# ed-fish/data-efficient-video-transformers

Hardware: AMD Instinct MI355X
Metric: clips/sec fwd+bwd, B=8 T=32 3x224x224 bf16 (higher is better)
Workload: dtype bf16; 1 GPU; ViViT metric shape (SURVEY 8 'M'; BASELINE configs[2]/[3] transformer): B=8/GPU, T=32, 3x224x224, patch 16, d=512, ...; global_batch=8, parallelism=dp1

## Files before the change

data-efficient-video-transformers_amd/csrc/attention.hip:

```cpp
#include "common.h"
#include <cstdlib>

namespace {

__device__ __forceinline__ void wave_lds_sync() {
  asm volatile("s_waitcnt lgkmcnt(0)" ::: "memory");
  __builtin_amdgcn_wave_barrier();
}

constexpr float kLog2e = 1.4426950408889634f;
constexpr float kLn2 = 0.6931471805599453f;

struct AttnParams {
  const void *q, *k, *v, *o, *d_o;
  void *out, *dq, *dk, *dv;
  float* lse;
  float* delta;
  int B, H, Lq, Lk, dh;
  int64_t q_sb, q_sh, q_sl, k_sb, k_sh, k_sl, v_sb, v_sh, v_sl, o_sb, o_sh, o_sl;
  float scale;
  int Lkp;
  int Lqp;
  int patch_off;
  uint32_t drop_thr;
  float drop_scale;
  const uint64_t* rng;
  uint64_t rng_off;
};


__device__ __forceinline__ float attn_drop(const AttnParams& p, int b, int h, int i, int j) {
  if (p.drop_thr == 0u) return 1.0f;
  const uint64_t idx = (((uint64_t)b * p.H + h) * p.Lq + i) * (uint64_t)p.Lk + j;
  return dvt_dropout_keep(p.rng[0], p.rng[1] + p.rng_off, idx, p.drop_thr) ? p.drop_scale : 0.0f;
}

template <typename T>
__global__ __launch_bounds__(256) void attn_fwd_generic_kernel(const AttnParams p) {
  extern __shared__ __attribute__((aligned(16))) float lds_f[];
  const int lane = threadIdx.x & 63, wid = threadIdx.x >> 6;
  float* qs = lds_f + (size_t)wid * (p.dh + p.Lk);
  float* ps = qs + p.dh;
  const int64_t row = (int64_t)blockIdx.x * 4 + wid;
  const int64_t total = (int64_t)p.B * p.H * p.Lq;
  if (row >= total) return;
  const int i = (int)(row % p.Lq);
  const int h = (int)((row / p.Lq) % p.H);
  const int b = (int)(row / ((int64_t)p.Lq * p.H));
  const T* q = (const T*)p.q + b * p.q_sb + h * p.q_sh + (int64_t)i * p.q_sl;
  const T* k = (const T*)p.k + b * p.k_sb + h * p.k_sh;
  const T* v = (const T*)p.v + b * p.v_sb + h * p.v_sh;
  T* o = (T*)p.out + b * p.o_sb + h * p.o_sh + (int64_t)i * p.o_sl;
  for (int e = lane; e < p.dh; e += 64) qs[e] = to_f32<T>(q[e]);
  wave_lds_sync();
  float m = -INFINITY;
  for (int j = lane; j < p.Lk; j += 64) {
    const T* kj = k + (int64_t)j * p.k_sl;
    float s = 0.f;
    for (int e = 0; e < p.dh; ++e) s = fmaf(qs[e], to_f32<T>(kj[e]), s);
    s *= p.scale;
    ps[j] = s;
    m = fmaxf(m, s);
  }
  m = wave_max(m);
  float l = 0.f;
  for (int j = lane; j < p.Lk; j += 64) {
    const float e = expf(ps[j] - m);
    ps[j] = e * attn_drop(p, b, h, i, j);
    l += e;
  }
  l = wave_sum(l);
  wave_lds_sync();
  const float inv = 1.0f / l;
  for (int e = lane; e < p.dh; e += 64) {
    float acc = 0.f;
    for (int j = 0; j < p.Lk; ++j) acc = fmaf(ps[j], to_f32<T>(v[(int64_t)j * p.v_sl + e]), acc);
    o[e] = from_f32<T>(acc * inv);
  }
  if (lane == 0) p.lse[row] = m + logf(l);
}

template <typename T>
__global__ __launch_bounds__(256) void attn_delta_kernel(const AttnParams p) {
  const int lane = threadIdx.x & 63, wid = threadIdx.x >> 6;
  const int64_t row = (int64_t)blockIdx.x * 4 + wid;
  const int64_t total = (int64_t)p.B * p.H * p.Lq;
  if (row >= total) return;
  const int i = (int)(row % p.Lq);
  const int h = (int)((row / p.Lq) % p.H);
  const int b = (int)(row / ((int64_t)p.Lq * p.H));
  const int64_t off = b * p.o_sb + h * p.o_sh + (int64_t)i * p.o_sl;
  const T* o = (const T*)p.o + off;
  const T* g = (const T*)p.d_o + off;
  float s = 0.f;
  for (int e = lane; e < p.dh; e += 64) s = fmaf(to_f32<T>(o[e]), to_f32<T>(g[e]), s);
  s = wave_sum(s);
  if (lane == 0) p.delta[row] = s;
}

template <typename T>
__global__ __launch_bounds__(256) void attn_bwd_dq_generic_kernel(const AttnParams p) {
  extern __shared__ __attribute__((aligned(16))) float lds_f[];
  const int lane = threadIdx.x & 63, wid = threadIdx.x >> 6;
  float* qs = lds_f + (size_t)wid * (2 * p.dh + p.Lk);
  float* gs = qs + p.dh;
  float* ds = gs + p.dh;
  const int64_t row = (int64_t)blockIdx.x * 4 + wid;
  const int64_t total = (int64_t)p.B * p.H * p.Lq;
  if (row >= total) return;
  const int i = (int)(row % p.Lq);
  const int h = (int)((row / p.Lq) % p.H);
  const int b = (int)(row / ((int64_t)p.Lq * p.H));
  const T* q = (const T*)p.q + b * p.q_sb + h * p.q_sh + (int64_t)i * p.q_sl;
  const T* g = (const T*)p.d_o + b * p.o_sb + h * p.o_sh + (int64_t)i * p.o_sl;
  const T* k = (const T*)p.k + b * p.k_sb + h * p.k_sh;
  const T* v = (const T*)p.v + b * p.v_sb + h * p.v_sh;
  T* dq = (T*)p.dq + b * p.q_sb + h * p.q_sh + (int64_t)i * p.q_sl;
  for (int e = lane; e < p.dh; e += 64) {
    qs[e] = to_f32<T>(q[e]);
    gs[e] = to_f32<T>(g[e]);
  }
  wave_lds_sync();
  const float lse = p.lse[row], delta = p.delta[row];
  for (int j = lane; j < p.Lk; j += 64) {
    const T* kj = k + (int64_t)j * p.k_sl;
    const T* vj = v + (int64_t)j * p.v_sl;
    float s = 0.f, dp = 0.f;
    for (int e = 0; e < p.dh; ++e) {
      s = fmaf(qs[e], to_f32<T>(kj[e]), s);
      dp = fmaf(gs[e], to_f32<T>(vj[e]), dp);
    }
    const float pr = expf(s * p.scale - lse);
    ds[j] = pr * (dp * attn_drop(p, b, h, i, j) - delta) * p.scale;
  }
  wave_lds_sync();
  for (int e = lane; e < p.dh; e += 64) {
    float acc = 0.f;
    for (int j = 0; j < p.Lk; ++j) acc = fmaf(ds[j], to_f32<T>(k[(int64_t)j * p.k_sl + e]), acc);
    dq[e] = from_f32<T>(acc);
  }
}

template <typename T>
__global__ __launch_bounds__(256) void attn_bwd_dkv_generic_kernel(const AttnParams p) {
  extern __shared__ __attribute__((aligned(16))) float lds_f[];
  const int lane = threadIdx.x & 63, wid = threadIdx.x >> 6;
  float* ks = lds_f + (size_t)wid * (2 * p.dh + 2 * p.Lq);
  float* vs = ks + p.dh;
  float* ps = vs + p.dh;
  float* ds = ps + p.Lq;
  const int64_t row = (int64_t)blockIdx.x * 4 + wid;
  const int64_t total = (int64_t)p.B * p.H * p.Lk;
  if (row >= total) return;
  const int j = (int)(row % p.Lk);
// ... 797 lines not shown
          const f32x2 ds = pr * d;
          s[tt][r] = ds[0];
          s[tt][r + 1] = ds[1];
          if (last && (2 * kp + tt) * 16 + 4 * g + r >= p.Lk) s[tt][r] = 0.f;
          if (last && (2 * kp + tt) * 16 + 4 * g + r + 1 >= p.Lk) s[tt][r + 1] = 0.f;
        }
      const V8 dsf = pack_pair<E>(s[0], s[1]);
#pragma unroll
      for (int dt = 0; dt < 4; ++dt)
        acc[dt] = Elem16<E>::mma(img_tr_frag<E>(ks, 2 * kp, 2 * kp + 1, dt * 16, g, li), dsf, acc[dt]);
    };
    if constexpr (NKP > 0) {
#pragma unroll
      for (int kp = 0; kp < NKP; ++kp) step(kp, kp == NKP - 1);
    } else {
      for (int kp = 0; kp < nkp - 1; ++kp) step(kp, false);
      step(nkp - 1, true);
    }
#pragma unroll
    for (int kk = 0; kk < 2; ++kk) {
      consume(qn[kk]);
      consume(gn[kk]);
      consume(of[kk]);
    }
    consume(l2n);
    store_tile<E>(patch, dqb, p.q_sl, qt * 16, p.Lq, acc, p.scale, lane);
#pragma unroll
    for (int kk = 0; kk < 2; ++kk) {
      qf[kk] = qn[kk];
      gf[kk] = gn[kk];
    }
    l2 = l2n;
  }
}

template <typename E, int NQP>
__global__ __launch_bounds__(1024) void attn_bwd_dkv_mfma_kernel(const AttnParams p) {
  extern __shared__ __attribute__((aligned(16))) char smem[];
  using V8 = typename Elem16<E>::v8;
  const int lane = threadIdx.x & 63, wid = threadIdx.x >> 6, W = blockDim.x >> 6;
  const int g = lane >> 4, li = lane & 15;
  const int b = blockIdx.x / p.H, h = blockIdx.x % p.H;
  const E* qb = (const E*)p.q + b * p.q_sb + h * p.q_sh;
  const E* kb = (const E*)p.k + b * p.k_sb + h * p.k_sh;
  const E* vb = (const E*)p.v + b * p.v_sb + h * p.v_sh;
  const E* gb = (const E*)p.d_o + b * p.o_sb + h * p.o_sh;
  E* dkb = (E*)p.dk + b * p.k_sb + h * p.k_sh;
  E* dvb = (E*)p.dv + b * p.v_sb + h * p.v_sh;
  const float* lse = p.lse + ((int64_t)b * p.H + h) * p.Lq;
  const float* delta = p.delta + ((int64_t)b * p.H + h) * p.Lq;
  char* qs = smem;
  char* gs = smem + p.Lqp * kRowBytes;
  float* l2s = reinterpret_cast<float*>(smem + 2 * p.Lqp * kRowBytes);
  float* dls = l2s + p.Lqp;
  const int nkt = (p.Lk + 15) >> 4, nqp = NQP ? NQP : p.Lqp >> 5;
  auto load_rows = [&](int kt, V8* kf, V8* vf) {
    const int kj = kt * 16 + li;
    const int krow = kj < p.Lk ? kj : p.Lk - 1;
#pragma unroll
    for (int kk = 0; kk < 2; ++kk) {
      kf[kk] = *reinterpret_cast<const V8*>(kb + (int64_t)krow * p.k_sl + kk * 32 + g * 8);
      vf[kk] = *reinterpret_cast<const V8*>(vb + (int64_t)krow * p.v_sl + kk * 32 + g * 8);
    }
  };
  V8 kf[2], vf[2];
  load_rows(wid, kf, vf);
  const int sr = (int)threadIdx.x < p.Lq ? (int)threadIdx.x : p.Lq - 1;
  const float lse0 = lse[sr], dl0 = delta[sr];
  stage_images<E>(qs, qb, p.q_sl, gs, gb, p.o_sl, p.Lq, p.Lqp);
  if ((int)threadIdx.x < p.Lqp) {
    l2s[threadIdx.x] = (int)threadIdx.x < p.Lq ? -lse0 * kLog2e : 0.f;
    dls[threadIdx.x] = (int)threadIdx.x < p.Lq ? -dl0 : 0.f;
  }
  for (int r = threadIdx.x + blockDim.x; r < p.Lqp; r += blockDim.x) {
    l2s[r] = r < p.Lq ? -lse[r] * kLog2e : 0.f;
    dls[r] = r < p.Lq ? -delta[r] : 0.f;
  }
  __syncthreads();

  const float c2 = p.scale * kLog2e;
  char* patch = p.patch_off >= 0 ? smem + p.patch_off + wid * 2048 : nullptr;
  for (int kt = wid; kt < nkt; kt += W) {
    asm volatile("" ::: "memory");
    f32x4 dk[4], dv[4];
#pragma unroll
    for (int dt = 0; dt < 4; ++dt) {
      dk[dt] = f32x4{0.f, 0.f, 0.f, 0.f};
      dv[dt] = f32x4{0.f, 0.f, 0.f, 0.f};
    }
    const f32x2 c2v = {c2, c2};
    auto step = [&](int qp) {
      f32x4 s[2], dp[2];
#pragma unroll
      for (int tt = 0; tt < 2; ++tt) {
        s[tt] = f32x4{0.f, 0.f, 0.f, 0.f};
        dp[tt] = f32x4{0.f, 0.f, 0.f, 0.f};
#pragma unroll
        for (int kk = 0; kk < 2; ++kk) {
          s[tt] = Elem16<E>::mma(img_row_frag<E>(qs, (2 * qp + tt) * 16, kk, g, li), kf[kk], s[tt]);
          dp[tt] = Elem16<E>::mma(img_row_frag<E>(gs, (2 * qp + tt) * 16, kk, g, li), vf[kk], dp[tt]);
        }
      }
#pragma unroll
      for (int tt = 0; tt < 2; ++tt) {
        const int q0 = (2 * qp + tt) * 16 + 4 * g;
        const f32x4 l2 = *reinterpret_cast<const f32x4*>(l2s + q0);
        const f32x4 dl = *reinterpret_cast<const f32x4*>(dls + q0);
#pragma unroll
        for (int r = 0; r < 4; r += 2) {
          const f32x2 x = __builtin_elementwise_fma(f32x2{s[tt][r], s[tt][r + 1]}, c2v, f32x2{l2[r], l2[r + 1]});
          const f32x2 d = f32x2{dp[tt][r], dp[tt][r + 1]} + f32x2{dl[r], dl[r + 1]};
          const f32x2 pr = {__builtin_amdgcn_exp2f(x[0]), __builtin_amdgcn_exp2f(x[1])};
          const f32x2 ds = pr * d;
          s[tt][r] = pr[0];
          s[tt][r + 1] = pr[1];
          dp[tt][r] = ds[0];
          dp[tt][r + 1] = ds[1];
        }
      }
      const V8 pf = pack_pair<E>(s[0], s[1]);
      const V8 dsf = pack_pair<E>(dp[0], dp[1]);
#pragma unroll
      for (int dt = 0; dt < 4; ++dt) {
        dv[dt] = Elem16<E>::mma(img_tr_frag<E>(gs, 2 * qp, 2 * qp + 1, dt * 16, g, li), pf, dv[dt]);
        dk[dt] = Elem16<E>::mma(img_tr_frag<E>(qs, 2 * qp, 2 * qp + 1, dt * 16, g, li), dsf, dk[dt]);
      }
    };
    if constexpr (NQP > 0) {
#pragma unroll
      for (int qp = 0; qp < NQP; ++qp) step(qp);
    } else {
      for (int qp = 0; qp < nqp; ++qp) step(qp);
    }
    if (kt + W < nkt) load_rows(kt + W, kf, vf);
    store_tile<E>(patch, dkb, p.k_sl, kt * 16, p.Lk, dk, p.scale, lane);
    store_tile<E>(patch, dvb, p.v_sl, kt * 16, p.Lk, dv, 1.0f, lane);
  }
}

constexpr int kStripRow = 80;

template <typename E>
__device__ __forceinline__ typename Elem16<E>::v8 strip_tr_frag(const char* strip, int ta, int tb, int col0, int g, int li) {
  const int qq = li >> 2, pp = li & 3;
  typename Elem16<E>::v4 half[2];
#pragma unroll
  for (int hf = 0; hf < 2; ++hf) {
    const int r = 16 * (hf ? tb : ta) + 4 * g + qq;
    half[hf] = Elem16<E>::tr_read(strip + r * kStripRow + col0 * 2 + 8 * pp);
  }
  return __builtin_shufflevector(half[0], half[1], 0, 1, 2, 3, 4, 5, 6, 7);
}

template <typename E, int NCH>
__device__ __forceinline__ void stage_bwd_operands(char* qs, const E* q, int64_t q_sl, char* gs, const E* g, const E* o, int64_t o_sl,
                                                   char* ks, const E* k, int64_t k_sl, int Lq, int Lk, int rows_pad, float* dls) {
  using V8 = typename Elem16<E>::v8;
  const int total = rows_pad * 8, nt = blockDim.x;
  V8 vq[NCH], vg[NCH], vo[NCH], vk[NCH];
#pragma unroll
  for (int u = 0; u < NCH; ++u) {
    const int idx = min((int)threadIdx.x + u * nt, total - 1);
    const int r = idx >> 3, c = idx & 7;
    const int rq = r < Lq ? r : 0, rk = r < Lk ? r : 0;
    vq[u] = *reinterpret_cast<const V8*>(q + (int64_t)rq * q_sl + c * 8);
    vg[u] = *reinterpret_cast<const V8*>(g + (int64_t)rq * o_sl + c * 8);
    vo[u] = *reinterpret_cast<const V8*>(o + (int64_t)rq * o_sl + c * 8);
    vk[u] = *reinterpret_cast<const V8*>(k + (int64_t)rk * k_sl + c * 8);
  }
  __builtin_amdgcn_sched_barrier(0);
  const V8 zero = {0, 0, 0, 0, 0, 0, 0, 0};
#pragma unroll
  for (int u = 0; u < NCH; ++u) {
    const int idx = min((int)threadIdx.x + u * nt, total - 1);
    const int r = idx >> 3, off = img_off(r, idx & 7);
    const bool lq = r < Lq, lk = r < Lk;
    *reinterpret_cast<V8*>(qs + off) = lq ? vq[u] : zero;
    *reinterpret_cast<V8*>(gs + off) = lq ? vg[u] : zero;
    *reinterpret_cast<V8*>(ks + off) = lk ? vk[u] : zero;
    float d = 0.f;
#pragma unroll
    for (int j = 0; j < 8; ++j) d = fmaf((float)vg[u][j], (float)vo[u][j], d);
    d += __shfl_xor(d, 1, 64);
    d += __shfl_xor(d, 2, 64);
    d += __shfl_xor(d, 4, 64);
    if ((idx & 7) == 0) dls[r] = lq ? -d : 0.f;
  }
}

template <typename E, int NP>
__global__ __launch_bounds__(512) void attn_bwd_fused_kernel(const AttnParams p) {
  extern __shared__ __attribute__((aligned(16))) char smem[];
  using V8 = typename Elem16<E>::v8;
  using V4 = typename Elem16<E>::v4;
  constexpr int LP = 32 * NP;
  const int lane = threadIdx.x & 63;
  const int wid = __builtin_amdgcn_readfirstlane(threadIdx.x >> 6);
  const int W = blockDim.x >> 6, WC = W - 1;
  const int g = lane >> 4, li = lane & 15;
  const int b = blockIdx.x / p.H, h = blockIdx.x % p.H;
  const E* qb = (const E*)p.q + b * p.q_sb + h * p.q_sh;
  const E* kb = (const E*)p.k + b * p.k_sb + h * p.k_sh;
  const E* vb = (const E*)p.v + b * p.v_sb + h * p.v_sh;
  const E* ob = (const E*)p.o + b * p.o_sb + h * p.o_sh;
  const E* gb = (const E*)p.d_o + b * p.o_sb + h * p.o_sh;
  E* dqb = (E*)p.dq + b * p.q_sb + h * p.q_sh;
  E* dkb = (E*)p.dk + b * p.k_sb + h * p.k_sh;
  E* dvb = (E*)p.dv + b * p.v_sb + h * p.v_sh;
  const float* lse = p.lse + ((int64_t)b * p.H + h) * p.Lq;
  char* qs = smem;
  char* gs = qs + LP * kRowBytes;
  char* ks = gs + LP * kRowBytes;
  char* strip0 = ks + LP * kRowBytes;
  float* l2s = reinterpret_cast<float*>(strip0 + 2 * LP * kStripRow);
  float* dls = l2s + LP;
  char* patch = reinterpret_cast<char*>(dls + LP) + wid * 2048;

  V8 kf[2][2], vf[2][2];
  if (wid < WC) {
#pragma unroll
    for (int j = 0; j < 2; ++j) {
      const int kj = (2 * wid + j) * 16 + li;
      const int krow = kj < p.Lk ? kj : p.Lk - 1;
#pragma unroll
      for (int kk = 0; kk < 2; ++kk) {
        kf[j][kk] = *reinterpret_cast<const V8*>(kb + (int64_t)krow * p.k_sl + kk * 32 + g * 8);
        vf[j][kk] = *reinterpret_cast<const V8*>(vb + (int64_t)krow * p.v_sl + kk * 32 + g * 8);
      }
    }
  }
  {
    const int r = threadIdx.x;
    const float l = lse[r < p.Lq ? r : 0];
    stage_bwd_operands<E, 4>(qs, qb, p.q_sl, gs, gb, ob, p.o_sl, ks, kb, p.k_sl, p.Lq, p.Lk, LP, dls);
    if (r < LP) l2s[r] = r < p.Lq ? -l * kLog2e : 0.f;
  }
  __syncthreads();
  const float c2 = p.scale * kLog2e;
  if (wid < WC) {
    f32x4 dk[2][4], dv[2][4];
#pragma unroll
    for (int j = 0; j < 2; ++j)
#pragma unroll
      for (int dt = 0; dt < 4; ++dt) {
        dk[j][dt] = f32x4{0.f, 0.f, 0.f, 0.f};
        dv[j][dt] = f32x4{0.f, 0.f, 0.f, 0.f};
      }
    const f32x2 c2v = {c2, c2};
    const bool kvalid[2] = {(2 * wid) * 16 + li < p.Lk, (2 * wid + 1) * 16 + li < p.Lk};
    char* myrow[2] = {strip0 + ((2 * wid) * 16 + li) * kStripRow + g * 8, strip0 + ((2 * wid + 1) * 16 + li) * kStripRow + g * 8};
#pragma unroll
    for (int qp = 0; qp < NP; ++qp) {
      asm volatile("" ::: "memory");
      V8 qfr[2][2], gfr[2][2];
#pragma unroll
      for (int tt = 0; tt < 2; ++tt)
#pragma unroll
        for (int kk = 0; kk < 2; ++kk) {
          qfr[tt][kk] = img_row_frag<E>(qs, (2 * qp + tt) * 16, kk, g, li);
          gfr[tt][kk] = img_row_frag<E>(gs, (2 * qp + tt) * 16, kk, g, li);
        }
      f32x4 l2[2], dl[2];
#pragma unroll
      for (int tt = 0; tt < 2; ++tt) {
        l2[tt] = *reinterpret_cast<const f32x4*>(l2s + (2 * qp + tt) * 16 + 4 * g);
        dl[tt] = *reinterpret_cast<const f32x4*>(dls + (2 * qp + tt) * 16 + 4 * g);
      }
      V8 pf[2], dsf[2];
#pragma unroll
      for (int j = 0; j < 2; ++j) {
        f32x4 s[2], dp[2];
#pragma unroll
        for (int tt = 0; tt < 2; ++tt) {
          s[tt] = f32x4{0.f, 0.f, 0.f, 0.f};
          dp[tt] = f32x4{0.f, 0.f, 0.f, 0.f};
#pragma unroll
          for (int kk = 0; kk < 2; ++kk) {
            s[tt] = Elem16<E>::mma(qfr[tt][kk], kf[j][kk], s[tt]);
            dp[tt] = Elem16<E>::mma(gfr[tt][kk], vf[j][kk], dp[tt]);
          }
        }
#pragma unroll
        for (int tt = 0; tt < 2; ++tt)
#pragma unroll
          for (int r = 0; r < 4; r += 2) {
            const f32x2 x = __builtin_elementwise_fma(f32x2{s[tt][r], s[tt][r + 1]}, c2v, f32x2{l2[tt][r], l2[tt][r + 1]});
            const f32x2 d = f32x2{dp[tt][r], dp[tt][r + 1]} + f32x2{dl[tt][r], dl[tt][r + 1]};
            f32x2 pr = {__builtin_amdgcn_exp2f(x[0]), __builtin_amdgcn_exp2f(x[1])};
            if (!kvalid[j]) pr = f32x2{0.f, 0.f};
            const f32x2 ds = pr * d;
            s[tt][r] = pr[0];
            s[tt][r + 1] = pr[1];
            dp[tt][r] = ds[0];
            dp[tt][r + 1] = ds[1];
          }
        pf[j] = pack_pair<E>(s[0], s[1]);
        dsf[j] = pack_pair<E>(dp[0], dp[1]);
      }
#pragma unroll
      for (int j = 0; j < 2; ++j) {
        char* row = myrow[j] + (qp & 1) * (LP * kStripRow);
        *reinterpret_cast<V4*>(row) = __builtin_shufflevector(dsf[j], dsf[j], 0, 1, 2, 3);
        *reinterpret_cast<V4*>(row + 32) = __builtin_shufflevector(dsf[j], dsf[j], 4, 5, 6, 7);
      }
#pragma unroll
      for (int dt = 0; dt < 4; ++dt) {
        const V8 gt = img_tr_frag<E>(gs, 2 * qp, 2 * qp + 1, dt * 16, g, li);
        const V8 qt = img_tr_frag<E>(qs, 2 * qp, 2 * qp + 1, dt * 16, g, li);
#pragma unroll
        for (int j = 0; j < 2; ++j) {
          dv[j][dt] = Elem16<E>::mma(gt, pf[j], dv[j][dt]);
          dk[j][dt] = Elem16<E>::mma(qt, dsf[j], dk[j][dt]);
        }
      }
      __syncthreads();
    }
#pragma unroll
    for (int j = 0; j < 2; ++j) {
      const int k0 = (2 * wid + j) * 16;
      if (k0 < p.Lk) {
        store_tile<E>(patch, dkb, p.k_sl, k0, p.Lk, dk[j], p.scale, lane);
        store_tile<E>(patch, dvb, p.v_sl, k0, p.Lk, dv[j], 1.0f, lane);
      }
    }
  } else {
    V8 ka[NP][4];
#pragma unroll
    for (int kp = 0; kp < NP; ++kp)
#pragma unroll
      for (int dt = 0; dt < 4; ++dt) ka[kp][dt] = img_tr_frag<E>(ks, 2 * kp, 2 * kp + 1, dt * 16, g, li);
#pragma unroll 1
    for (int qp = 0; qp < NP; ++qp) {
      __syncthreads();
      const char* strip = strip0 + (qp & 1) * (LP * kStripRow);
      V8 bq[NP][2];
#pragma unroll
      for (int kp = 0; kp < NP; ++kp) {
        bq[kp][0] = strip_tr_frag<E>(strip, 2 * kp, 2 * kp + 1, 0, g, li);
        bq[kp][1] = strip_tr_frag<E>(strip, 2 * kp, 2 * kp + 1, 16, g, li);
      }
      f32x4 acc[2][4];
#pragma unroll
      for (int tt = 0; tt < 2; ++tt)
#pragma unroll
        for (int dt = 0; dt < 4; ++dt) acc[tt][dt] = f32x4{0.f, 0.f, 0.f, 0.f};
#pragma unroll
      for (int kp = 0; kp < NP; ++kp)
#pragma unroll
        for (int dt = 0; dt < 4; ++dt) {
          acc[0][dt] = Elem16<E>::mma(ka[kp][dt], bq[kp][0], acc[0][dt]);
          acc[1][dt] = Elem16<E>::mma(ka[kp][dt], bq[kp][1], acc[1][dt]);
        }
#pragma unroll
      for (int tt = 0; tt < 2; ++tt)
        if ((2 * qp + tt) * 16 < p.Lq) store_tile<E>(nullptr, dqb, p.q_sl, (2 * qp + tt) * 16, p.Lq, acc[tt], p.scale, lane);
    }
  }
}

constexpr int kMaxLds = 160 * 1024;

int fill_params(const dvt_attn_desc* d, AttnParams& p, bool bwd, const char* name) {
  DVT_REQUIRE(d, "%s: null descriptor", name);
  DVT_REQUIRE(d->q && d->k && d->v && d->o && d->lse, "%s: null q/k/v/o/lse", name);
  DVT_REQUIRE(d->B >= 0 && d->H > 0 && d->Lq > 0 && d->Lk > 0 && d->dh > 0, "%s: bad sizes", name);
  DVT_REQUIRE(d->B * d->H < (1ll << 31) && d->Lq < (1 << 24) && d->Lk < (1 << 24), "%s: sizes too large", name);
  if (bwd) DVT_REQUIRE(d->d_o && d->dq && d->dk && d->dv, "%s: null gradient pointer", name);
  p.q = d->q; p.k = d->k; p.v = d->v; p.o = d->o; p.out = d->o; p.d_o = d->d_o;
  p.dq = d->dq; p.dk = d->dk; p.dv = d->dv; p.lse = d->lse; p.delta = nullptr;
  p.B = (int)d->B; p.H = (int)d->H; p.Lq = (int)d->Lq; p.Lk = (int)d->Lk; p.dh = (int)d->dh;
  p.q_sb = d->q_sb; p.q_sh = d->q_sh; p.q_sl = d->q_sl;
  p.k_sb = d->k_sb; p.k_sh = d->k_sh; p.k_sl = d->k_sl;
  p.v_sb = d->v_sb; p.v_sh = d->v_sh; p.v_sl = d->v_sl;
  p.o_sb = d->o_sb; p.o_sh = d->o_sh; p.o_sl = d->o_sl;
  p.scale = d->scale;
  DVT_REQUIRE(d->dropout_p >= 0.f && d->dropout_p < 1.f, "%s: dropout_p must be in [0, 1)", name);
  DVT_REQUIRE(d->dropout_p == 0.f || d->rng_state, "%s: dropout needs rng_state", name);
  p.drop_thr = 0u; p.drop_scale = 1.f; p.rng = d->rng_state; p.rng_off = d->rng_offset;
  if (d->dropout_p > 0.f) {
    const double th = (double)d->dropout_p * 4294967296.0;
    p.drop_thr = th >= 4294967295.0 ? 0xFFFFFFFFu : (uint32_t)(th + 0.5);
    if (p.drop_thr == 0u) p.drop_thr = 1u;
    p.drop_scale = 1.0f / (1.0f - d->dropout_p);
  }
  p.Lkp = (p.Lk + 31) & ~31;
  p.Lqp = (p.Lq + 31) & ~31;
  p.patch_off = -1;

  return DVT_OK;
}

bool strides_vec_ok(const dvt_attn_desc* d) {
  const int64_t s[] = {d->q_sb, d->q_sh, d->q_sl, d->k_sb, d->k_sh, d->k_sl,
                       d->v_sb, d->v_sh, d->v_sl, d->o_sb, d->o_sh, d->o_sl};
  for (int64_t x : s)
    if (x % 8) return false;
  return true;
}

bool mfma_fwd_ok(const dvt_attn_desc* d, const AttnParams& p) {
  return d->dropout_p == 0.f && d->scale > 0.f && dvt_is_16bit(d->dtype) && d->dh == DH && strides_vec_ok(d) && dvt_aligned16(d->q) &&
         dvt_aligned16(d->k) && dvt_aligned16(d->v) && dvt_aligned16(d->o) &&
         2 * p.Lkp * kRowBytes <= kMaxLds;
}

bool q1_ok(const dvt_attn_desc* d, const AttnParams& p) {
  return p.Lq == 1 && d->dropout_p == 0.f && dvt_is_16bit(d->dtype) && d->dh == DH && strides_vec_ok(d) &&
         dvt_aligned16(d->q) && dvt_aligned16(d->k) && dvt_aligned16(d->v) && dvt_aligned16(d->o) &&
         (size_t)4 * p.Lkp * sizeof(float) <= (size_t)kMaxLds;
}

bool mfma_bwd_ok(const dvt_attn_desc* d, const AttnParams& p) {
  return mfma_fwd_ok(d, p) && dvt_aligned16(d->d_o) && dvt_aligned16(d->dq) && dvt_aligned16(d->dk) &&
         dvt_aligned16(d->dv) && 2 * p.Lqp * kRowBytes + 2 * p.Lqp * 4 <= kMaxLds;
}

bool fused_bwd_ok(const AttnParams& p) { return p.Lqp == p.Lkp && p.Lkp <= 224; }
size_t fused_bwd_lds(int NP, int waves) {
  const size_t LP = 32 * (size_t)NP;
  return 3 * LP * kRowBytes + 2 * LP * kStripRow + 2 * LP * sizeof(float) + (size_t)waves * 2048;
}

int pick_waves(int tiles, size_t lds_bytes, int cap = 16) {
  int maxw = lds_bytes > 80 * 1024 ? 16 : 8;
  if (maxw > cap) maxw = cap;
  const int rounds = (tiles + maxw - 1) / maxw;
  int w = (tiles + rounds - 1) / rounds;
  return w < 1 ? 1 : w;
}

size_t with_patches(size_t lds, int waves, AttnParams& p) {
  const size_t tot = lds + (size_t)waves * 2048;
  const bool ok = lds <= 80 * 1024 ? 2 * tot <= (size_t)kMaxLds : tot <= (size_t)kMaxLds;
  p.patch_off = ok ? (int)lds : -1;
  return ok ? tot : lds;
}

template <typename K>
int set_lds(K kernel, size_t bytes) {
  if (bytes > 64 * 1024) {
    const hipError_t e = hipFuncSetAttribute((const void*)kernel, hipFuncAttributeMaxDynamicSharedMemorySize, (int)bytes);
    if (e != hipSuccess) return dvt_fail_hip(e, "hipFuncSetAttribute(MaxDynamicSharedMemorySize)");
  }
  return 0;
}

int resolve_fwd(const dvt_attn_desc* d, AttnParams& p, dvt_attn_plan_info& r) {
  r = dvt_attn_plan_info{};
  r.patch = r.patch2 = -1;
  int rc = fill_params(d, p, false, "dvt_attention_fwd");
  if (rc) return rc;
  if (p.B == 0) return DVT_OK;
  if (q1_ok(d, p)) {
    r.family = DVT_ATTN_F_Q1; r.waves = 4; r.lds = (int64_t)4 * p.Lkp * sizeof(float);
    return DVT_OK;
  }
  if (mfma_fwd_ok(d, p)) {
    const size_t lds_img = (size_t)2 * p.Lkp * kRowBytes;
    const int nkp = p.Lkp >> 5;
    r.waves = pick_waves((p.Lq + 15) / 16, lds_img, nkp > 7 && nkp <= 11 ? 12 : 16);
    r.lds = (int64_t)with_patches(lds_img, r.waves, p);
    r.patch = p.patch_off >= 0;
    r.family = nkp <= 11 ? DVT_ATTN_F_RES : DVT_ATTN_F_ONLINE;
    r.count = nkp <= 11 ? nkp : 0;
    return DVT_OK;
  }
  const int nt_s = p.Lq * p.dh >= 4096 ? 512 : 256;
  const size_t lds_s = ((size_t)(p.Lq + 2 * p.Lk) * small_dhp(p.dh) +
                        (size_t)small_parts(p.Lq, p.Lk, nt_s) * p.Lq * small_lp(p.Lk)) * sizeof(float);
  if (d->dtype != DVT_F32 && d->dtype != DVT_BF16 && d->dtype != DVT_F16)
    DVT_UNSUPPORTED("dvt_attention_fwd: dtype %d not supported", d->dtype);
  if (p.Lq <= kSmallL && p.Lk <= kSmallL && p.dh <= kSmallDh && lds_s <= (size_t)kMaxLds) {
    r.family = DVT_ATTN_F_SMALL; r.waves = nt_s / 64; r.lds = (int64_t)lds_s;
    return DVT_OK;
  }
  const size_t lds = (size_t)4 * (p.dh + p.Lk) * sizeof(float);
  if (lds > (size_t)kMaxLds) DVT_UNSUPPORTED("dvt_attention_fwd: Lk = %d, dh = %d exceed the LDS budget", p.Lk, p.dh);
  r.family = DVT_ATTN_F_GENERIC; r.waves = 4; r.lds = (int64_t)lds;
// ... 244 lines not shown
```

Baseline: 1454 clips/s.

## Stream Q/dO/O strips per step in fused attention backward and specialize partial KV tiles

The fused attention backward kernel no longer stages all of Q, dO, O and K into LDS upfront with every thread. Compute waves now load Q/dO/O strips in 32-row chunks, double-buffered in registers and landed one step ahead for large NP. The dQ wave loads K into LDS itself. The change also swaps the light wave's KV block assignment, skips the dead second tile through a compile-time NJ=1 path, and adds waves_per_eu occupancy hints. The aim is to overlap global loads with MFMA work and cut the initial staging stall, at the cost of more register pressure and more complex synchronisation.

```diff
diff --git a/data-efficient-video-transformers_amd/csrc/attention.hip b/data-efficient-video-transformers_amd/csrc/attention.hip
--- a/data-efficient-video-transformers_amd/csrc/attention.hip
+++ b/data-efficient-video-transformers_amd/csrc/attention.hip
@@ -1,5 +1,6 @@
 #include "common.h"
 #include <cstdlib>
+#include <type_traits>
 
 namespace {
 
@@ -1103,32 +1104,38 @@
   return __builtin_shufflevector(half[0], half[1], 0, 1, 2, 3, 4, 5, 6, 7);
 }
 
-template <typename E, int NCH>
-__device__ __forceinline__ void stage_bwd_operands(char* qs, const E* q, int64_t q_sl, char* gs, const E* g, const E* o, int64_t o_sl,
-                                                   char* ks, const E* k, int64_t k_sl, int Lq, int Lk, int rows_pad, float* dls) {
+constexpr int kStripChunks = 32 * 8;
+
+template <typename E, int NCH, int NS>
+__device__ __forceinline__ void strip_request(typename Elem16<E>::v8 (&vq)[NS * NCH], typename Elem16<E>::v8 (&vg)[NS * NCH],
+                                              typename Elem16<E>::v8 (&vo)[NS * NCH], const E* q, int64_t q_sl, const E* g,
+                                              const E* o, int64_t o_sl, int s, int Lq, int ct, int nt) {
   using V8 = typename Elem16<E>::v8;
-  const int total = rows_pad * 8, nt = blockDim.x;
-  V8 vq[NCH], vg[NCH], vo[NCH], vk[NCH];
-#pragma unroll
-  for (int u = 0; u < NCH; ++u) {
-    const int idx = min((int)threadIdx.x + u * nt, total - 1);
-    const int r = idx >> 3, c = idx & 7;
-    const int rq = r < Lq ? r : 0, rk = r < Lk ? r : 0;
+#pragma unroll
+  for (int u = 0; u < NS * NCH; ++u) {
+    const int idx = min(ct + (u % NCH) * nt, kStripChunks - 1);
+    const int r = 32 * (s + u / NCH) + (idx >> 3), c = idx & 7;
+    const int rq = r < Lq ? r : 0;
     vq[u] = *reinterpret_cast<const V8*>(q + (int64_t)rq * q_sl + c * 8);
     vg[u] = *reinterpret_cast<const V8*>(g + (int64_t)rq * o_sl + c * 8);
     vo[u] = *reinterpret_cast<const V8*>(o + (int64_t)rq * o_sl + c * 8);
-    vk[u] = *reinterpret_cast<const V8*>(k + (int64_t)rk * k_sl + c * 8);
   }
   __builtin_amdgcn_sched_barrier(0);
+}
+
+template <typename E, int NCH, int NS>
+__device__ __forceinline__ void strip_land(const typename Elem16<E>::v8 (&vq)[NS * NCH], const typename Elem16<E>::v8 (&vg)[NS * NCH],
+                                           const typename Elem16<E>::v8 (&vo)[NS * NCH], char* qs, char* gs, float* dls, int s,
+                                           int Lq, int ct, int nt) {
+  using V8 = typename Elem16<E>::v8;
   const V8 zero = {0, 0, 0, 0, 0, 0, 0, 0};
 #pragma unroll
-  for (int u = 0; u < NCH; ++u) {
-    const int idx = min((int)threadIdx.x + u * nt, total - 1);
-    const int r = idx >> 3, off = img_off(r, idx & 7);
-    const bool lq = r < Lq, lk = r < Lk;
+  for (int u = 0; u < NS * NCH; ++u) {
+    const int idx = min(ct + (u % NCH) * nt, kStripChunks - 1);
+    const int r = 32 * (s + u / NCH) + (idx >> 3), off = img_off(r, idx & 7);
+    const bool lq = r < Lq;
     *reinterpret_cast<V8*>(qs + off) = lq ? vq[u] : zero;
     *reinterpret_cast<V8*>(gs + off) = lq ? vg[u] : zero;
-    *reinterpret_cast<V8*>(ks + off) = lk ? vk[u] : zero;
     float d = 0.f;
 #pragma unroll
     for (int j = 0; j < 8; ++j) d = fmaf((float)vg[u][j], (float)vo[u][j], d);
@@ -1139,7 +1146,11 @@
   }
 }
 
+template <int NP>
+constexpr int fused_bwd_light_wave() { return NP >= 4 ? NP - 4 : NP - 1; }
+
 template <typename E, int NP>
+__attribute__((amdgpu_waves_per_eu(NP == 1 ? 4 : NP <= 4 ? 3 : 2)))
 __global__ __launch_bounds__(512) void attn_bwd_fused_kernel(const AttnParams p) {
   extern __shared__ __attribute__((aligned(16))) char smem[];
   using V8 = typename Elem16<E>::v8;
@@ -1167,11 +1178,20 @@
   float* dls = l2s + LP;
   char* patch = reinterpret_cast<char*>(dls + LP) + wid * 2048;
 
-  V8 kf[2][2], vf[2][2];
+  const float c2 = p.scale * kLog2e;
+  constexpr int NCH = (kStripChunks + 64 * NP - 1) / (64 * NP);
+  constexpr bool kStream = NP >= 5;
+  constexpr int NS0 = kStream ? 1 : NP;
   if (wid < WC) {
+    constexpr int LW = fused_bwd_light_wave<NP>();
+    const int blk = wid == LW ? NP - 1 : wid == NP - 1 ? LW : wid;
+    const bool live1 = (2 * blk + 1) * 16 < p.Lk;
+    const bool carry = NP <= 4 || wid * 64 < kStripChunks;
+    const int ct = threadIdx.x, nt = 64 * WC;
+    V8 kf[2][2], vf[2][2];
 #pragma unroll
     for (int j = 0; j < 2; ++j) {
-      const int kj = (2 * wid + j) * 16 + li;
+      const int kj = (2 * blk + j) * 16 + li;
       const int krow = kj < p.Lk ? kj : p.Lk - 1;
 #pragma unroll
       for (int kk = 0; kk < 2; ++kk) {
@@ -1179,16 +1199,22 @@
         vf[j][kk] = *reinterpret_cast<const V8*>(vb + (int64_t)krow * p.v_sl + kk * 32 + g * 8);
       }
     }
-  }
-  {
-    const int r = threadIdx.x;
-    const float l = lse[r < p.Lq ? r : 0];
-    stage_bwd_operands<E, 4>(qs, qb, p.q_sl, gs, gb, ob, p.o_sl, ks, kb, p.k_sl, p.Lq, p.Lk, LP, dls);
-    if (r < LP) l2s[r] = r < p.Lq ? -l * kLog2e : 0.f;
-  }
-  __syncthreads();
-  const float c2 = p.scale * kLog2e;
-  if (wid < WC) {
+    const float l = lse[ct < p.Lq ? ct : 0];
+    V8 sq[2][NS0 * NCH], sg[2][NS0 * NCH], so[2][NS0 * NCH];
+    strip_request<E, NCH, NS0>(sq[0], sg[0], so[0], qb, p.q_sl, gb, ob, p.o_sl, 0, p.Lq, ct, nt);
+    if constexpr (kStream) strip_request<E, NCH, NS0>(sq[1], sg[1], so[1], qb, p.q_sl, gb, ob, p.o_sl, 1, p.Lq, ct, nt);
+    char* myrow[2] = {strip0 + ((2 * blk) * 16 + li) * kStripRow + g * 8, strip0 + ((2 * blk + 1) * 16 + li) * kStripRow + g * 8};
+    if (!live1) {
+      const V4 z4 = {0, 0, 0, 0};
+#pragma unroll
+      for (int sb = 0; sb < 2; ++sb) {
+        *reinterpret_cast<V4*>(myrow[1] + sb * (LP * kStripRow)) = z4;
+        *reinterpret_cast<V4*>(myrow[1] + sb * (LP * kStripRow) + 32) = z4;
+      }
+    }
+    if (ct < LP) l2s[ct] = ct < p.Lq ? -l * kLog2e : 0.f;
+    if (carry) strip_land<E, NCH, NS0>(sq[0], sg[0], so[0], qs, gs, dls, 0, p.Lq, ct, nt);
+    __syncthreads();
     f32x4 dk[2][4], dv[2][4];
 #pragma unroll
     for (int j = 0; j < 2; ++j)
@@ -1198,11 +1224,16 @@
         dv[j][dt] = f32x4{0.f, 0.f, 0.f, 0.f};
       }
     const f32x2 c2v = {c2, c2};
-    const bool kvalid[2] = {(2 * wid) * 16 + li < p.Lk, (2 * wid + 1) * 16 + li < p.Lk};
-    char* myrow[2] = {strip0 + ((2 * wid) * 16 + li) * kStripRow + g * 8, strip0 + ((2 * wid + 1) * 16 + li) * kStripRow + g * 8};
+    const bool kvalid[2] = {(2 * blk) * 16 + li < p.Lk, (2 * blk + 1) * 16 + li < p.Lk};
+    auto steps = [&](auto nj) {
+    constexpr int NJ = decltype(nj)::value;
 #pragma unroll
     for (int qp = 0; qp < NP; ++qp) {
       asm volatile("" ::: "memory");
+      if constexpr (kStream)
+        if (qp + 2 < NP) {
+          strip_request<E, NCH, NS0>(sq[qp & 1], sg[qp & 1], so[qp & 1], qb, p.q_sl, gb, ob, p.o_sl, qp + 2, p.Lq, ct, nt);
+        }
       V8 qfr[2][2], gfr[2][2];
 #pragma unroll
       for (int tt = 0; tt < 2; ++tt)
@@ -1217,9 +1248,9 @@
         l2[tt] = *reinterpret_cast<const f32x4*>(l2s + (2 * qp + tt) * 16 + 4 * g);
         dl[tt] = *reinterpret_cast<const f32x4*>(dls + (2 * qp + tt) * 16 + 4 * g);
       }
-      V8 pf[2], dsf[2];
-#pragma unroll
-      for (int j = 0; j < 2; ++j) {
+      V8 pf[NJ], dsf[NJ];
+#pragma unroll
+      for (int j = 0; j < NJ; ++j) {
         f32x4 s[2], dp[2];
 #pragma unroll
         for (int tt = 0; tt < 2; ++tt) {
@@ -1249,7 +1280,7 @@
         dsf[j] = pack_pair<E>(dp[0], dp[1]);
       }
 #pragma unroll
-      for (int j = 0; j < 2; ++j) {
+      for (int j = 0; j < NJ; ++j) {
         char* row = myrow[j] + (qp & 1) * (LP * kStripRow);
         *reinterpret_cast<V4*>(row) = __builtin_shufflevector(dsf[j], dsf[j], 0, 1, 2, 3);
         *reinterpret_cast<V4*>(row + 32) = __builtin_shufflevector(dsf[j], dsf[j], 4, 5, 6, 7);
@@ -1259,22 +1290,41 @@
         const V8 gt = img_tr_frag<E>(gs, 2 * qp, 2 * qp + 1, dt * 16, g, li);
         const V8 qt = img_tr_frag<E>(qs, 2 * qp, 2 * qp + 1, dt * 16, g, li);
 #pragma unroll
-        for (int j = 0; j < 2; ++j) {
+        for (int j = 0; j < NJ; ++j) {
           dv[j][dt] = Elem16<E>::mma(gt, pf[j], dv[j][dt]);
           dk[j][dt] = Elem16<E>::mma(qt, dsf[j], dk[j][dt]);
         }
       }
+      if constexpr (kStream)
+        if (qp + 1 < NP && carry) {
+          strip_land<E, NCH, NS0>(sq[(qp + 1) & 1], sg[(qp + 1) & 1], so[(qp + 1) & 1], qs, gs, dls, qp + 1, p.Lq, ct, nt);
+        }
       __syncthreads();
     }
+    };
+    if (live1) steps(std::integral_constant<int, 2>{}); else steps(std::integral_constant<int, 1>{});
 #pragma unroll
     for (int j = 0; j < 2; ++j) {
-      const int k0 = (2 * wid + j) * 16;
+      const int k0 = (2 * blk + j) * 16;
       if (k0 < p.Lk) {
         store_tile<E>(patch, dkb, p.k_sl, k0, p.Lk, dk[j], p.scale, lane);
         store_tile<E>(patch, dvb, p.v_sl, k0, p.Lk, dv[j], 1.0f, lane);
       }
     }
   } else {
+    V8 vk[4 * NP];
+#pragma unroll
+    for (int u = 0; u < 4 * NP; ++u) {
+      const int r = 8 * u + (lane >> 3);
+      vk[u] = *reinterpret_cast<const V8*>(kb + (int64_t)(r < p.Lk ? r : 0) * p.k_sl + (lane & 7) * 8);
+    }
+    __builtin_amdgcn_sched_barrier(0);
+    __syncthreads();
+#pragma unroll
+    for (int u = 0; u < 4 * NP; ++u) {
+      const int r = 8 * u + (lane >> 3);
+      *reinterpret_cast<V8*>(ks + img_off(r, lane & 7)) = r < p.Lk ? vk[u] : V8{0, 0, 0, 0, 0, 0, 0, 0};
+    }
     V8 ka[NP][4];
 #pragma unroll
     for (int kp = 0; kp < NP; ++kp)
```

New measurement: 1461 clips/s, median of 3. No clear change (+0.5%).
